# peternara/FashionVisualExpl-recommend

Hardware: AMD Instinct MI355X
Metric: BPR triplets/sec (higher is better)
Workload: dtype bf16

## Files before the change

fashionvisualexpl_recommend_amd/csrc/bprx_philox.hip:

```cpp
#include <hip/hip_runtime.h>

#include "bprx_internal.h"

namespace {


__device__ __forceinline__ int32_t nth_non_positive(const int32_t *__restrict__ lst, long long len, uint32_t I, uint32_t z,
                                                    int32_t last) {
  long long distinct = 0;
  for (long long q = 0; q < len; ++q) distinct += (q == 0 || lst[q] != lst[q - 1]);
  if (distinct >= (long long)I) return last;
  uint32_t x = __umulhi(z, I - (uint32_t)distinct);
  for (long long q = 0; q < len; ++q) {
    if (q && lst[q] == lst[q - 1]) continue;
    if ((uint32_t)lst[q] <= x) ++x; else break;
  }
  return x < I ? (int32_t)x : last;
}

__device__ __forceinline__ void put_planes(uint8_t *__restrict__ own8, uint8_t *__restrict__ loc8, long long pi, long long pj,
                                           int32_t ii, int32_t jj, int sh) {
  own8[pi] = (uint8_t)(ii >> sh); own8[pj] = (uint8_t)(jj >> sh);
  if (sh == 8) { loc8[pi] = (uint8_t)ii; loc8[pj] = (uint8_t)jj; }
  else {
    uint16_t *l16 = reinterpret_cast<uint16_t *>(loc8);
    const int m = (1 << sh) - 1;
    l16[pi] = (uint16_t)(ii & m); l16[pj] = (uint16_t)(jj & m);
  }
}

__global__ __launch_bounds__(256) void k_sample_philox(const int64_t *__restrict__ indptr, const int32_t *__restrict__ items,
                                                       const int32_t *__restrict__ pos_user, unsigned long long N, uint32_t I,
                                                       uint32_t k0, uint32_t k1, unsigned long long first, long long B,
                                                       int32_t *__restrict__ u, int32_t *__restrict__ i, int32_t *__restrict__ j,
                                                       uint8_t *__restrict__ own8, uint8_t *__restrict__ loc8, long long pl_i,
                                                       long long pl_j, int sh) {
  const long long b = (long long)blockIdx.x * 256 + threadIdx.x;
  if (b >= B) return;
  const unsigned long long n = first + (unsigned long long)b;
  uint32_t r[4];
  philox4x32_10((uint32_t)n, (uint32_t)(n >> 32), 0u, 0u, k0, k1, r);
  const unsigned long long x = ((unsigned long long)r[1] << 32) | r[0];
  const unsigned long long p = __umul64hi(x, N);
  const int32_t uu = pos_user[p];
  const long long lo0 = indptr[uu], len = indptr[uu + 1] - lo0;
  const int32_t *lst = items + lo0;
  int32_t jj = 0;
  bool hit = true;
  for (uint32_t a = 0; a < 1024u && hit; ++a) {
    if (a) philox4x32_10((uint32_t)n, (uint32_t)(n >> 32), a, 0u, k0, k1, r);
    jj = (int32_t)__umulhi(r[2], I);
    long long lo = 0, hi = len;
    while (lo < hi) {
      const long long mid = (lo + hi) >> 1;
      if (lst[mid] < jj) lo = mid + 1; else hi = mid;
    }
    hit = lo < len && lst[lo] == jj;
  }
  if (hit) {
    philox4x32_10((uint32_t)n, (uint32_t)(n >> 32), 1024u, 0u, k0, k1, r);
    jj = nth_non_positive(lst, len, I, r[2], jj);
  }
  const int32_t ii = items[p];
  u[b] = uu; i[b] = ii; j[b] = jj;
  if (own8) put_planes(own8, loc8, pl_i + b, pl_j + b, ii, jj, sh);
}

__global__ __launch_bounds__(256) void k_sample_epoch(const int64_t *__restrict__ indptr, const int32_t *__restrict__ items,
                                                      const int32_t *__restrict__ perm, const int64_t *__restrict__ epoch_ptr,
                                                      const int32_t *__restrict__ pos_slot, int U, uint32_t I, uint32_t k0, uint32_t k1, uint32_t epoch,
                                                      long long first, long long B, int32_t *__restrict__ u,
                                                      int32_t *__restrict__ i, int32_t *__restrict__ j,
                                                      uint8_t *__restrict__ own8, uint8_t *__restrict__ loc8, long long pl_i,
                                                      long long pl_j, int sh) {
  const long long b = (long long)blockIdx.x * 256 + threadIdx.x;
  if (b >= B) return;
  const long long n = first + b;
  int lo = 0, hi = U;
  if (pos_slot) lo = pos_slot[n];
  else
    while (hi - lo > 1) {
      const int mid = (lo + hi) >> 1;
      if (epoch_ptr[mid] <= n) lo = mid; else hi = mid;
    }
  const int32_t uu = perm[lo];
  const long long l0 = indptr[uu], len = indptr[uu + 1] - l0;
  const int32_t *lst = items + l0;
  uint32_t r[4];
  int32_t jj = 0;
  bool hit = true;
  for (uint32_t a = 0; a < 1024u && hit; ++a) {
    philox4x32_10((uint32_t)n, (uint32_t)((unsigned long long)n >> 32), a, epoch, k0, k1, r);
    jj = (int32_t)__umulhi(r[2], I);
    long long l = 0, h = len;
    while (l < h) {
      const long long mid = (l + h) >> 1;
      if (lst[mid] < jj) l = mid + 1; else h = mid;
    }
    hit = l < len && lst[l] == jj;
  }
  if (hit) {
    philox4x32_10((uint32_t)n, (uint32_t)((unsigned long long)n >> 32), 1024u, epoch, k0, k1, r);
    jj = nth_non_positive(lst, len, I, r[2], jj);
  }
  const int32_t ii = lst[n - epoch_ptr[lo]];
  u[b] = uu; i[b] = ii; j[b] = jj;
  if (own8) put_planes(own8, loc8, pl_i + b, pl_j + b, ii, jj, sh);
}

__device__ __forceinline__ uint32_t epoch_perm_at(uint32_t a, uint32_t U, int half, uint32_t k0, uint32_t k1, uint32_t epoch) {
  const uint32_t mask = (1u << half) - 1u;
  uint32_t x = a;
  do {
    uint32_t L = x >> half, R = x & mask;
#pragma unroll
    for (uint32_t r = 0; r < 4; ++r) {
      uint32_t o[4];
      philox4x32_10(R, r, 0xFFFFFFFEu, epoch, k0, k1, o);
      const uint32_t t = L ^ (o[0] & mask);
      L = R; R = t;
    }
    x = (L << half) | R;
  } while (x >= U);
  return x;
}

__host__ __device__ inline int epoch_perm_half(uint32_t U) {
  int nb = 1;
  while (nb < 32 && (U - 1u) >> nb) ++nb;
  return (nb + 1) / 2;
}

__global__ __launch_bounds__(256) void k_epoch_prepare(uint32_t k0, uint32_t k1, uint32_t epoch, int U, int half,
                                                       const int64_t *__restrict__ indptr, int32_t *__restrict__ perm,
                                                       int64_t *__restrict__ lens) {
  const int a = blockIdx.x * 256 + threadIdx.x;
  if (a >= U) return;
  const uint32_t u = epoch_perm_at((uint32_t)a, (uint32_t)U, half, k0, k1, epoch);
  perm[a] = (int32_t)u;
  lens[a] = indptr[u + 1] - indptr[u];
}

__global__ __launch_bounds__(256) void k_epoch_slots(const int64_t *__restrict__ epoch_ptr, int U, int32_t *__restrict__ pos_slot,
                                                     int64_t num_pos) {
  const int a = (blockIdx.x * 256 + threadIdx.x) >> 3, lane = threadIdx.x & 7;
  if (a >= U) return;
  const int64_t p0 = epoch_ptr[a];
  int64_t p1 = epoch_ptr[a + 1];
  p1 = p1 < num_pos ? p1 : num_pos;
  for (int64_t p = p0 + lane; p < p1; p += 8) pos_slot[p] = a;
}

}

extern "C" int bprx_epoch_prepare(uint64_t seed, uint32_t epoch, int32_t num_users, const int64_t *indptr, int32_t *perm,
                                  int64_t *lens, void *stream) {
  if (!indptr || !perm || !lens || num_users <= 0) return BPRX_E_INVALID;
  hipLaunchKernelGGL(k_epoch_prepare, dim3((unsigned)((num_users + 255) / 256)), dim3(256), 0, (hipStream_t)stream, (uint32_t)seed,
                     (uint32_t)(seed >> 32), epoch, num_users, epoch_perm_half((uint32_t)num_users), indptr, perm, lens);
  return hipGetLastError() == hipSuccess ? BPRX_OK : BPRX_E_HIP;
}

extern "C" int bprx_epoch_slots(const int64_t *epoch_ptr, int32_t num_users, int32_t *pos_slot, int64_t num_pos, void *stream) {
  if (!epoch_ptr || !pos_slot || num_users <= 0 || num_pos < 0) return BPRX_E_INVALID;
  hipLaunchKernelGGL(k_epoch_slots, dim3((unsigned)(((int64_t)num_users * 8 + 255) / 256)), dim3(256), 0, (hipStream_t)stream,
                     epoch_ptr, num_users, pos_slot, num_pos);
  return hipGetLastError() == hipSuccess ? BPRX_OK : BPRX_E_HIP;
}

static void plane_args(bprx_handle *h, const int32_t *pos, const int32_t *neg, int64_t B, int64_t batch_offset, int64_t batch_size,
                       uint8_t **own8, uint8_t **loc8, long long *pl_i, long long *pl_j, int *sh) {
  *own8 = nullptr; *loc8 = nullptr; *pl_i = 0; *pl_j = 0; *sh = 8;
  if (!h || !h->own8 || batch_size <= 0 || batch_size > h->cfg.max_batch || batch_offset < 0 || batch_offset + B > batch_size) return;
  if (batch_offset == 0) { h->idx8_pos = pos; h->idx8_neg = neg; h->idx8_B = batch_size; h->idx8_n = 0; }
  else if (h->idx8_n < 0 || h->idx8_B != batch_size || pos != h->idx8_pos + batch_offset || neg != h->idx8_neg + batch_offset) {
    h->idx8_n = -1;
    return;
  }
  h->idx8_n += B;
  *own8 = h->own8; *loc8 = h->loc8; *pl_i = batch_offset; *pl_j = batch_size + batch_offset; *sh = h->idx8_shift;
}

extern "C" int bprx_sample_epoch_h(bprx_handle *h, const int64_t *indptr, const int32_t *items_sorted, const int32_t *perm,
                                   const int64_t *epoch_ptr, const int32_t *pos_slot, int32_t num_users, int32_t num_items,
                                   uint64_t seed, uint32_t epoch, int64_t first, int64_t B, int32_t *user, int32_t *pos, int32_t *neg,
                                   int64_t batch_offset, int64_t batch_size, void *stream) {
  if (!indptr || !items_sorted || !perm || !epoch_ptr || !user || !pos || !neg || num_users <= 0 || num_items <= 0 ||
      B < 0 || first < 0)
    return BPRX_E_INVALID;
  if (B == 0) return BPRX_OK;
  uint8_t *own8, *loc8;
  long long pl_i, pl_j;
  int sh;
  plane_args(h, pos, neg, B, batch_offset, batch_size, &own8, &loc8, &pl_i, &pl_j, &sh);
  hipLaunchKernelGGL(k_sample_epoch, dim3((unsigned)((B + 255) / 256)), dim3(256), 0, (hipStream_t)stream, indptr,
                     items_sorted, perm, epoch_ptr, pos_slot, num_users, (uint32_t)num_items, (uint32_t)seed, (uint32_t)(seed >> 32),
                     epoch, (long long)first, (long long)B, user, pos, neg, own8, loc8, pl_i, pl_j, sh);
  return hipGetLastError() == hipSuccess ? BPRX_OK : BPRX_E_HIP;
}

extern "C" int bprx_sample_epoch(const int64_t *indptr, const int32_t *items_sorted, const int32_t *perm,
                                 const int64_t *epoch_ptr, const int32_t *pos_slot, int32_t num_users, int32_t num_items, uint64_t seed,
                                 uint32_t epoch, int64_t first, int64_t B, int32_t *user, int32_t *pos, int32_t *neg,
                                 void *stream) {
  return bprx_sample_epoch_h(nullptr, indptr, items_sorted, perm, epoch_ptr, pos_slot, num_users, num_items, seed, epoch, first, B,
                             user, pos, neg, 0, 0, stream);
}

extern "C" int bprx_sample_philox_h(bprx_handle *h, const int64_t *indptr, const int32_t *items_sorted, const int32_t *pos_user,
                                    int64_t num_pos, int32_t num_items, uint64_t seed, uint64_t first, int64_t B, int32_t *user,
                                    int32_t *pos, int32_t *neg, int64_t batch_offset, int64_t batch_size, void *stream) {
  if (!indptr || !items_sorted || !pos_user || !user || !pos || !neg || num_pos <= 0 || num_items <= 0 || B < 0)
    return BPRX_E_INVALID;
  if (B == 0) return BPRX_OK;
  uint8_t *own8, *loc8;
  long long pl_i, pl_j;
  int sh;
  plane_args(h, pos, neg, B, batch_offset, batch_size, &own8, &loc8, &pl_i, &pl_j, &sh);
  hipLaunchKernelGGL(k_sample_philox, dim3((unsigned)((B + 255) / 256)), dim3(256), 0, (hipStream_t)stream, indptr,
                     items_sorted, pos_user, (unsigned long long)num_pos, (uint32_t)num_items, (uint32_t)seed,
                     (uint32_t)(seed >> 32), (unsigned long long)first, (long long)B, user, pos, neg, own8, loc8, pl_i, pl_j, sh);
  return hipGetLastError() == hipSuccess ? BPRX_OK : BPRX_E_HIP;
}

extern "C" int bprx_sample_philox(const int64_t *indptr, const int32_t *items_sorted, const int32_t *pos_user,
                                  int64_t num_pos, int32_t num_items, uint64_t seed, uint64_t first, int64_t B,
                                  int32_t *user, int32_t *pos, int32_t *neg, void *stream) {
  return bprx_sample_philox_h(nullptr, indptr, items_sorted, pos_user, num_pos, num_items, seed, first, B, user, pos, neg, 0, 0,
                              stream);
}
```

Before: 315.7 million.

## Preload short user item lists into registers for negative-sample membership tests

```diff
diff --git a/fashionvisualexpl_recommend_amd/csrc/bprx_philox.hip b/fashionvisualexpl_recommend_amd/csrc/bprx_philox.hip
--- a/fashionvisualexpl_recommend_amd/csrc/bprx_philox.hip
+++ b/fashionvisualexpl_recommend_amd/csrc/bprx_philox.hip
@@ -18,6 +18,49 @@
   return x < I ? (int32_t)x : last;
 }
 
+constexpr int LIST_REGS = 32;
+
+__device__ __forceinline__ int wave_list_bound(long long len, bool live) {
+  int m = live ? (int)(len < (long long)LIST_REGS ? len : (long long)LIST_REGS) : 0;
+#pragma unroll
+  for (int o = 32; o > 0; o >>= 1) { const int t = __shfl_xor(m, o, 64); m = t > m ? t : m; }
+  return __builtin_amdgcn_readfirstlane(m);
+}
+
+__device__ __forceinline__ void list_request(const int32_t *__restrict__ items, long long l0, long long len, int wmax,
+                                             int32_t (&v)[LIST_REGS]) {
+  const int32_t *base = len > 0 ? items + l0 : items;
+  const int last = len > 0 ? (int)((len < (long long)LIST_REGS ? len : (long long)LIST_REGS) - 1) : 0;
+#pragma unroll
+  for (int q = 0; q < LIST_REGS; ++q) v[q] = -1;
+#pragma unroll
+  for (int g = 0; g < LIST_REGS; g += 8)
+    if (g < wmax) {
+#pragma unroll
+      for (int q = g; q < g + 8; ++q) v[q] = base[q < last ? q : last];
+    }
+}
+
+__device__ __forceinline__ void list_mask(long long len, int32_t (&v)[LIST_REGS]) {
+#pragma unroll
+  for (int q = 0; q < LIST_REGS; ++q) v[q] = (long long)q < len ? v[q] : -1;
+}
+
+__device__ __forceinline__ bool list_has(const int32_t (&v)[LIST_REGS], const int32_t *__restrict__ lst, long long len, int32_t jj) {
+  if (len <= (long long)LIST_REGS) {
+    bool hit = false;
+#pragma unroll
+    for (int q = 0; q < LIST_REGS; ++q) hit |= v[q] == jj;
+    return hit;
+  }
+  long long lo = 0, hi = len;
+  while (lo < hi) {
+    const long long mid = (lo + hi) >> 1;
+    if (lst[mid] < jj) lo = mid + 1; else hi = mid;
+  }
+  return lo < len && lst[lo] == jj;
+}
+
 __device__ __forceinline__ void put_planes(uint8_t *__restrict__ own8, uint8_t *__restrict__ loc8, long long pi, long long pj,
                                            int32_t ii, int32_t jj, int sh) {
   own8[pi] = (uint8_t)(ii >> sh); own8[pj] = (uint8_t)(jj >> sh);
@@ -35,33 +78,33 @@
                                                        int32_t *__restrict__ u, int32_t *__restrict__ i, int32_t *__restrict__ j,
                                                        uint8_t *__restrict__ own8, uint8_t *__restrict__ loc8, long long pl_i,
                                                        long long pl_j, int sh) {
-  const long long b = (long long)blockIdx.x * 256 + threadIdx.x;
-  if (b >= B) return;
+  const long long b0 = (long long)blockIdx.x * 256 + threadIdx.x;
+  const bool live = b0 < B;
+  const long long b = live ? b0 : B - 1;
   const unsigned long long n = first + (unsigned long long)b;
   uint32_t r[4];
   philox4x32_10((uint32_t)n, (uint32_t)(n >> 32), 0u, 0u, k0, k1, r);
   const unsigned long long x = ((unsigned long long)r[1] << 32) | r[0];
   const unsigned long long p = __umul64hi(x, N);
   const int32_t uu = pos_user[p];
+  const int32_t ii = items[p];
   const long long lo0 = indptr[uu], len = indptr[uu + 1] - lo0;
   const int32_t *lst = items + lo0;
+  int32_t v[LIST_REGS];
+  list_request(items, lo0, len, wave_list_bound(len, live), v);
+  list_mask(len, v);
   int32_t jj = 0;
   bool hit = true;
   for (uint32_t a = 0; a < 1024u && hit; ++a) {
     if (a) philox4x32_10((uint32_t)n, (uint32_t)(n >> 32), a, 0u, k0, k1, r);
     jj = (int32_t)__umulhi(r[2], I);
-    long long lo = 0, hi = len;
-    while (lo < hi) {
-      const long long mid = (lo + hi) >> 1;
-      if (lst[mid] < jj) lo = mid + 1; else hi = mid;
-    }
-    hit = lo < len && lst[lo] == jj;
+    hit = list_has(v, lst, len, jj);
   }
   if (hit) {
     philox4x32_10((uint32_t)n, (uint32_t)(n >> 32), 1024u, 0u, k0, k1, r);
     jj = nth_non_positive(lst, len, I, r[2], jj);
   }
-  const int32_t ii = items[p];
+  if (!live) return;
   u[b] = uu; i[b] = ii; j[b] = jj;
   if (own8) put_planes(own8, loc8, pl_i + b, pl_j + b, ii, jj, sh);
 }
@@ -73,8 +116,9 @@
                                                       int32_t *__restrict__ i, int32_t *__restrict__ j,
                                                       uint8_t *__restrict__ own8, uint8_t *__restrict__ loc8, long long pl_i,
                                                       long long pl_j, int sh) {
-  const long long b = (long long)blockIdx.x * 256 + threadIdx.x;
-  if (b >= B) return;
+  const long long b0 = (long long)blockIdx.x * 256 + threadIdx.x;
+  const bool live = b0 < B;
+  const long long b = live ? b0 : B - 1;
   const long long n = first + b;
   int lo = 0, hi = U;
   if (pos_slot) lo = pos_slot[n];
@@ -84,26 +128,26 @@
       if (epoch_ptr[mid] <= n) lo = mid; else hi = mid;
     }
   const int32_t uu = perm[lo];
+  const long long e0 = epoch_ptr[lo];
   const long long l0 = indptr[uu], len = indptr[uu + 1] - l0;
   const int32_t *lst = items + l0;
+  const int32_t ii = lst[n - e0];
+  int32_t v[LIST_REGS];
+  list_request(items, l0, len, wave_list_bound(len, live), v);
+  list_mask(len, v);
   uint32_t r[4];
   int32_t jj = 0;
   bool hit = true;
   for (uint32_t a = 0; a < 1024u && hit; ++a) {
     philox4x32_10((uint32_t)n, (uint32_t)((unsigned long long)n >> 32), a, epoch, k0, k1, r);
     jj = (int32_t)__umulhi(r[2], I);
-    long long l = 0, h = len;
-    while (l < h) {
-      const long long mid = (l + h) >> 1;
-      if (lst[mid] < jj) l = mid + 1; else h = mid;
-    }
-    hit = l < len && lst[l] == jj;
+    hit = list_has(v, lst, len, jj);
   }
   if (hit) {
     philox4x32_10((uint32_t)n, (uint32_t)((unsigned long long)n >> 32), 1024u, epoch, k0, k1, r);
     jj = nth_non_positive(lst, len, I, r[2], jj);
   }
-  const int32_t ii = lst[n - epoch_ptr[lo]];
+  if (!live) return;
   u[b] = uu; i[b] = ii; j[b] = jj;
   if (own8) put_planes(own8, loc8, pl_i + b, pl_j + b, ii, jj, sh);
 }
```

After: 316.3 million, median of 3. About the same (+0.2%).
